# OmerKerner/noLZSS

Measured on AMD Instinct MI355X. Metric: bases/sec factorized (1 GB sigma=4 DNA) + HBM GB/s fraction, higher is better.
Workload: dtype u32; 1 GPU; dna1g: one 2^30-base synthetic DNA sequence per GPU (sigma=4, 40% copied blocks, 1% substitutions), full factorization to (start,length,ref) records in HBM; bases_per_gpu=1073741824, parallelism=1 independent sequence shard(s), all-gather of counts

## Files before the change

nolzss_amd/csrc/lpnf.hip:

```cpp
#include "pipeline.hpp"

#include <cstdlib>
#include "nearest_lds.hpp"
#include "queues.hpp"
#include "text_order.hpp"
#include "scan.hpp"

namespace nolzss {

__global__ void shard_totals_kernel(const uint32_t *const *counts, int nq, uint32_t *totals) {
    const int q = blockIdx.x;
    if (q >= nq) return;
    uint32_t v = threadIdx.x < kQShards ? counts[q][threadIdx.x * kQPad] : 0u;
    v = wave_reduce(v, OpAdd<uint32_t>());
    __shared__ uint32_t s_part[kQShards / 64];
    if (lane_id() == 0) s_part[threadIdx.x >> 6] = v;
    __syncthreads();
    if (threadIdx.x == 0) {
        uint32_t t = 0;
        for (uint32_t k = 0; k < kQShards / 64; ++k) t += s_part[k];
        totals[q] = t;
    }
}

namespace {

constexpr int kThreads = 256;
constexpr uint32_t kFarBothUnknown = 0xfffffffeu;

__device__ __forceinline__ bool lpf_decide(uint32_t i, uint32_t lp, uint32_t jp, uint32_t ls, uint32_t js,
                                           uint32_t *__restrict__ dst) {
    const uint32_t M = lp > ls ? lp : ls;
    if (M == 0) {
        *dst = 0;
        return false;
    }
    const bool ok = (lp == M && i - jp >= M) || (ls == M && i - js >= M);
    if (ok) {
        *dst = M;
        return false;
    }
    uint32_t lo = 0;
    if (lp > 0) { const uint32_t c = lp < i - jp ? lp : i - jp; lo = c > lo ? c : lo; }
    if (ls > 0) { const uint32_t c = ls < i - js ? ls : i - js; lo = c > lo ? c : lo; }
    *dst = lo;
    return true;
}

template <bool kTimed>
__global__ __launch_bounds__(kLdsThreads) void lpf_tile_kernel(const uint32_t *__restrict__ sa,
                                                               const uint32_t *__restrict__ lcp, uint32_t n,
                                                               uint32_t *__restrict__ lstar_by_rank,
                                                               ShardQueue exact_q, uint32_t *__restrict__ far_items,
                                                               uint32_t *__restrict__ far_cnt,
                                                               uint32_t *__restrict__ far_aux,
                                                               unsigned long long *__restrict__ phases,
                                                               uint32_t *__restrict__ psa1, uint32_t *__restrict__ plcp1,
                                                               uint32_t pending_min, uint32_t *__restrict__ pending_flag) {
    constexpr int NS = 2;
    const bool timed = kTimed && phases != nullptr && (blockIdx.x & 15) == 0;
    unsigned long long clk[6] = {0, 0, 0, 0, 0, 0};
    if (timed) clk[0] = __builtin_readcyclecounter();
    __shared__ __align__(16) uint32_t s_sa[kLdsSpan];
    __shared__ __align__(16) uint32_t s_lcp[kLdsSpan + 4];
    __shared__ uint32_t s_len[NS * kLdsTile];
    __shared__ uint16_t s_pos[NS * kLdsTile];
    constexpr int kListCapB = 64;
    __shared__ uint16_t s_list0[kLdsWaves][NS * kLdsPerWave];
    __shared__ uint16_t s_list1[kLdsWaves][NS * kListCapB];
    __shared__ uint32_t s_blk[3 * kBlkTableLen];
    const uint32_t base = blockIdx.x * (uint32_t)kLdsTile;
    const uint32_t shard = blockIdx.x % kQShards;
    stage_tile(sa, lcp, n, base, s_sa, s_lcp, pending_min, pending_flag);
    __syncthreads();
    const BlockTables T = block_tables<false>(s_blk);
    build_block_tables<false>(s_sa, s_lcp, T);
    __syncthreads();
    if (psa1 != nullptr && threadIdx.x < kLdsTile / kBlk) {
        const uint32_t B = (uint32_t)kLdsReach / kBlk + threadIdx.x;
        const uint64_t first = (uint64_t)base + (uint64_t)threadIdx.x * kBlk;
        if (first + kBlk <= (uint64_t)n) {
            psa1[first >> 4] = T.mn[B];
            plcp1[first >> 4] = T.ldn[B];
        }
    }
    if (timed) clk[1] = __builtin_readcyclecounter();
    const int w = threadIdx.x >> 6;
    const uint32_t far_bit = n <= 0x80000000u ? 0x80000000u : 0u;
    lds_search_wave_blocks<NS, NS, false, kLdsPerWave, kListCapB>(s_sa, s_lcp, T, n, base, s_len, s_pos, s_list0[w], s_list1[w],
                                   [](uint32_t) { return true; }, [](uint32_t) { return 0u; }, far_bit,
                                   timed ? clk + 2 : nullptr);
    if (timed) clk[4] = __builtin_readcyclecounter();
    constexpr int kRows = kLdsPerWave / 64;
    bool far[kRows], exact[kRows];
    uint32_t aux[kRows], known[kRows], fslot[kRows], eslot[kRows];
#pragma unroll
    for (int row = 0; row < kRows; ++row) {
        const int t = w * kLdsPerWave + row * 64 + lane_id();
        const uint64_t rr = (uint64_t)base + t;
        const bool in = rr < n;
        uint32_t up = s_len[t], down = s_len[kLdsTile + t];
        const bool fu = far_is(up, far_bit), fd = far_is(down, far_bit);
        far[row] = far_resolve(up, down, far_bit, 0u) && in;
        exact[row] = false;
        aux[row] = kFarBothUnknown;
        known[row] = 0;
        if (far[row]) {
            if (far_bit && fu != fd) {
                known[row] = fu ? down : up;
                const uint32_t p = match_pos(s_sa, fu ? s_pos[kLdsTile + t] : s_pos[t]);
                aux[row] = (known[row] ? (p & 0x7fffffffu) : 0x7fffffffu) | (fu ? 0x80000000u : 0u);
            }
        } else if (in) {
            exact[row] = lpf_decide(s_sa[t + kLdsReach], up, match_pos(s_sa, s_pos[t]), down, match_pos(s_sa, s_pos[kLdsTile + t]),
                                    lstar_by_rank + rr);
        }
    }
    {
        const uint32_t region = (blockIdx.x * (uint32_t)kLdsWaves + (uint32_t)w);
        uint32_t used = 0;
#pragma unroll
        for (int row = 0; row < kRows; ++row) {
            const uint64_t bal = __ballot(far[row]);
            fslot[row] = region * (uint32_t)kLdsPerWave + used + (uint32_t)__popcll(bal & lanemask_lt());
            used += (uint32_t)__popcll(bal);
        }
        if (lane_id() == 0) far_cnt[region] = used;
    }
    shard_slots<kRows>(exact_q, shard, exact, eslot);
#pragma unroll
    for (int row = 0; row < kRows; ++row) {
        const int t = w * kLdsPerWave + row * 64 + lane_id();
        const uint64_t rr = (uint64_t)base + t;
        if (far[row]) {
            far_items[fslot[row]] = (uint32_t)rr;
            lstar_by_rank[rr] = known[row];
            far_aux[rr] = aux[row];
        }
        if (exact[row]) exact_q.items[eslot[row]] = s_sa[t + kLdsReach];
    }
    if (timed) {
        __builtin_amdgcn_s_waitcnt(0);
        clk[5] = __builtin_readcyclecounter();
        if (lane_id() == 0) {
            for (int k = 0; k < 5; ++k) atomicAdd(phases + k, clk[k + 1] - clk[k]);
            atomicAdd(phases + 5, 1ull);
        }
    }
}

__global__ __launch_bounds__(kThreads) void compact_far_kernel(const uint32_t *__restrict__ far_items,
                                                               const uint32_t *__restrict__ far_cnt,
                                                               const uint32_t *__restrict__ far_off, uint32_t regions,
                                                               uint32_t *__restrict__ far_list) {
    const size_t stride = (size_t)gridDim.x * blockDim.x / 4;
    for (size_t r = ((size_t)blockIdx.x * blockDim.x + threadIdx.x) / 4; r < regions; r += stride) {
        const uint32_t c = far_cnt[r], o = far_off[r];
        for (uint32_t k = threadIdx.x & 3u; k < c; k += 4) far_list[o + k] = far_items[r * (size_t)kLdsPerWave + k];
    }
}

__global__ __launch_bounds__(kThreads) void lpf_far_kernel(const uint32_t *__restrict__ far_list, uint32_t far_count,
                                                           const uint32_t *__restrict__ sa,
                                                           const uint32_t *__restrict__ lcp, uint32_t n,
                                                           Pyramid Psa, Pyramid Plcp,
                                                           const uint32_t *__restrict__ by_rank,
                                                           const uint32_t *__restrict__ far_aux, bool bounded,
                                                           uint32_t *__restrict__ lstar, uint32_t *__restrict__ far_exact) {
    const size_t stride = (size_t)gridDim.x * blockDim.x;
    for (size_t k = (size_t)blockIdx.x * blockDim.x + threadIdx.x; k < far_count; k += stride) {
        const uint32_t r = far_list[k];
        const uint32_t i = sa[r];
        const uint32_t aux = far_aux[r];
        uint32_t lp, jp, ls, js;
        if (!bounded) {
            nearest_up<false>(sa, lcp, Psa, Plcp, r, i, 0u, lp, jp);
            nearest_down<false>(sa, lcp, n, Psa, Plcp, r, i, lp, ls, js);
        } else if (aux == kFarBothUnknown) {
            far_up<false>(sa, Psa, Plcp, r, i, 0u, lp, jp);
            far_down<false>(sa, n, Psa, Plcp, r, i, lp, ls, js);
        } else if (aux >> 31) {
            ls = by_rank[r];
            js = (aux & 0x7fffffffu) == 0x7fffffffu ? kNoPos : (aux & 0x7fffffffu);
            far_up<false>(sa, Psa, Plcp, r, i, ls, lp, jp);
        } else {
            lp = by_rank[r];
            jp = (aux & 0x7fffffffu) == 0x7fffffffu ? kNoPos : (aux & 0x7fffffffu);
            far_down<false>(sa, n, Psa, Plcp, r, i, lp, ls, js);
        }
        far_exact[k] = lpf_decide(i, lp, jp, ls, js, lstar + i) ? i : kNoPos;
    }
}

__global__ __launch_bounds__(kThreads) void lpnf_fallback_list_kernel(const uint32_t *__restrict__ far_exact,
                                                                      uint32_t far_count, uint32_t n,
                                                                      const uint32_t *__restrict__ isa, Pyramid Psa,
                                                                      Pyramid Plcp, uint32_t *__restrict__ lstar) {
    const size_t stride = (size_t)gridDim.x * blockDim.x;
    for (size_t k = (size_t)blockIdx.x * blockDim.x + threadIdx.x; k < far_count; k += stride) {
        const uint32_t i = far_exact[k];
        if (i == kNoPos) continue;
        const uint32_t cap = (n - i) < i ? (n - i) : i;
        lstar[i] = lpnf_search(Psa, Plcp, isa[i] - 1u, i, lstar[i], cap);
    }
}

__global__ __launch_bounds__(kThreads) void lpnf_fallback_kernel(ShardQueue exact_q, uint32_t n,
                                                                 const uint32_t *__restrict__ isa,
                                                                 Pyramid Psa, Pyramid Plcp,
                                                                 uint32_t *__restrict__ lstar) {
    const uint32_t shard = blockIdx.x;
    const uint32_t count = exact_q.counts[shard * kQPad];
    const uint32_t *items = exact_q.items + (size_t)shard * exact_q.cap;
    for (uint32_t k = blockIdx.y * blockDim.x + threadIdx.x; k < count; k += gridDim.y * blockDim.x) {
        const uint32_t i = items[k];
        const uint32_t cap = (n - i) < i ? (n - i) : i;
        lstar[i] = lpnf_search(Psa, Plcp, isa[i] - 1u, i, lstar[i], cap);
    }
}

}

uint32_t build_lstar(Context &ctx, uint32_t n, const uint32_t *sa, const uint32_t *isa, const uint32_t *lcp,
                     const Pyramid &Psa, const Pyramid &Plcp, uint32_t *lstar, uint32_t *isa_fill,
                     const PackedText *fill_pyramids) {
    hipStream_t s = ctx.stream;
    const size_t mark = ctx.arena.mark();
    uint32_t *pending_flag = nullptr;
    if (fill_pyramids) {
        pending_flag = ctx.arena.alloc<uint32_t>(1);
        HIP_CHECK(hipMemsetAsync(pending_flag, 0, sizeof(uint32_t), s));
        inject_pending_for_test(ctx, const_cast<uint32_t *>(lcp), n);
    }
    uint32_t *psa1 = fill_pyramids && Psa.nlev > 1 ? const_cast<uint32_t *>(Psa.lvl[1]) : nullptr;
    uint32_t *plcp1 = fill_pyramids && Plcp.nlev > 1 ? const_cast<uint32_t *>(Plcp.lvl[1]) : nullptr;
    if (!psa1 || !plcp1) psa1 = plcp1 = nullptr;
    const unsigned tiles = (unsigned)div_up(n, kLdsTile);
    ShardQueue exact_q;
    exact_q.cap = (uint32_t)shard_queue_cap(tiles, kLdsTile);
    exact_q.items = ctx.arena.alloc<uint32_t>((size_t)kQShards * exact_q.cap);
    const uint32_t far_regions = tiles * (uint32_t)kLdsWaves;
    uint32_t *far_items = ctx.arena.alloc<uint32_t>((size_t)far_regions * kLdsPerWave);
    uint32_t *far_cnt = ctx.arena.alloc<uint32_t>(far_regions);
    uint32_t *far_off = ctx.arena.alloc<uint32_t>(far_regions);
    uint32_t *qcounts = ctx.arena.alloc<uint32_t>(kQShards * kQPad);
    exact_q.counts = qcounts;
    const uint32_t **count_ptrs = ctx.arena.alloc<const uint32_t *>(1);
    uint32_t *totals = ctx.arena.alloc<uint32_t>(2);
    uint32_t *by_rank = ctx.arena.alloc<uint32_t>(n);
    uint32_t *far_aux = ctx.arena.alloc<uint32_t>(n);
    uint32_t *scratch_idx = ctx.arena.alloc<uint32_t>(n);
    uint32_t *scratch_val = ctx.arena.alloc<uint32_t>(isa_fill ? 2 * (size_t)n : (size_t)n);
    HIP_CHECK(hipMemsetAsync(qcounts, 0, kQShards * kQPad * sizeof(uint32_t), s));
    const uint32_t *h_ptrs[1] = {exact_q.counts};
    HIP_CHECK(hipMemcpyAsync(count_ptrs, h_ptrs, sizeof h_ptrs, hipMemcpyHostToDevice, s));
    HIP_CHECK(hipStreamSynchronize(s));
    auto read_totals = [&](uint32_t h[2]) {
        shard_totals_kernel<<<1, kQShards, 0, s>>>(count_ptrs, 1, totals);
        KERNEL_CHECK();
        ctx.read_back(totals, h, 2);
    };
    {
        ProfScope ps(ctx.profiler(), "lpf", s, 12.0 * (double)n);
        static const bool want_phases = getenv("NOLZSS_LPF_PHASES") != nullptr;
        unsigned long long *phases = nullptr;
        if (want_phases) {
            phases = ctx.arena.alloc<unsigned long long>(8);
            HIP_CHECK(hipMemsetAsync(phases, 0, 64, s));
        }
        if (phases)
            lpf_tile_kernel<true><<<tiles, kLdsThreads, 0, s>>>(sa, lcp, n, by_rank, exact_q, far_items, far_cnt, far_aux, phases, psa1, plcp1,
                                                                pending_threshold(), pending_flag);
        else
            lpf_tile_kernel<false><<<tiles, kLdsThreads, 0, s>>>(sa, lcp, n, by_rank, exact_q, far_items, far_cnt, far_aux, nullptr, psa1,
                                                                 plcp1, pending_threshold(), pending_flag);
        KERNEL_CHECK();
        if (phases) {
            unsigned long long h[8];
            HIP_CHECK(hipMemcpyAsync(h, phases, 64, hipMemcpyDeviceToHost, s));
            HIP_CHECK(hipStreamSynchronize(s));
            const double w = h[5] ? (double)h[5] : 1.0;
            fprintf(stderr, "[nolzss] lpf_tile phases (cycles per wavefront, %llu sampled): stage %.0f  round0 %.0f  %s %.0f  %s %.0f  epilogue %.0f\n",
                    h[5], h[0] / w, h[1] / w, "roundA", h[2] / w, "roundsBC", h[3] / w, h[4] / w);
        }
    }
    scan_exclusive_add_u32(far_cnt, far_off, far_regions, totals + 1, ctx.arena, s);
    if (fill_pyramids) {
        ProfScope ps(ctx.profiler(), "pyramids", s);
        if (psa1) {
            fill_pyramid_tail(Psa, n >> kPyrShift, false, s);
            fill_pyramid_tail(Plcp, n >> kPyrShift, false, s);
            fill_pyramid(Psa, 2, false, s);
            fill_pyramid(Plcp, 2, false, s);
        } else {
            fill_pyramid(Psa, 1, false, s);
            fill_pyramid(Plcp, 1, false, s);
        }
        uint32_t pending = 0;
        ctx.read_back(pending_flag, &pending, 1);
        if (pending) {
            ctx.arena.rewind(mark);
            finish_pending_lcp(ctx, *fill_pyramids, sa, const_cast<uint32_t *>(lcp));
            fill_pyramid(Psa, 1, false, s);
            fill_pyramid(Plcp, 1, false, s);
            return build_lstar(ctx, n, sa, isa, lcp, Psa, Plcp, lstar, isa_fill, nullptr);
        }
    }
    {
        ProfScope ps(ctx.profiler(), "lpf_to_text_order", s);
        uint32_t *idx[2] = {const_cast<uint32_t *>(sa), scratch_idx};
        uint32_t *val[2] = {by_rank, scratch_val};
        bucketed_scatter(idx, val, n, lstar, n, ctx.arena, s, ctx.profiler(), true, true, ctx.rec_plan, isa_fill);
    }
    uint32_t h[2] = {0, 0};
    read_totals(h);
    static const bool trace = getenv("NOLZSS_TRACE") != nullptr;
    if (trace) fprintf(stderr, "[nolzss] lpf: %u ranks to the far queue, %u positions to the exact search so far\n", h[1], h[0]);
    if (h[1] > 0) {
        ProfScope ps(ctx.profiler(), "lpf_far", s);
        uint32_t *far_list = ctx.arena.alloc<uint32_t>(h[1]);
        compact_far_kernel<<<(unsigned)std::min<size_t>(div_up((size_t)far_regions * 4, kThreads), 256u * 16u), kThreads, 0, s>>>(
            far_items, far_cnt, far_off, far_regions, far_list);
        KERNEL_CHECK();
        uint32_t *far_exact = ctx.arena.alloc<uint32_t>(h[1]);
        const unsigned g = (unsigned)std::min<size_t>(256u * 64u, std::max<size_t>(1, div_up(h[1], kThreads)));
        lpf_far_kernel<<<g, kThreads, 0, s>>>(far_list, h[1], sa, lcp, n, Psa, Plcp, by_rank, far_aux, n <= 0x80000000u,
                                              lstar, far_exact);
        KERNEL_CHECK();
        lpnf_fallback_list_kernel<<<g, kThreads, 0, s>>>(far_exact, h[1], n, isa, Psa, Plcp, lstar);
        KERNEL_CHECK();
    }
    if (h[0] > 0) {
        ProfScope ps(ctx.profiler(), "lpnf_fallback", s);
        const unsigned gy = (unsigned)std::min<size_t>(64, std::max<size_t>(1, div_up(h[0], (size_t)kQShards * kThreads)));
        lpnf_fallback_kernel<<<dim3(kQShards, gy), kThreads, 0, s>>>(exact_q, n, isa, Psa, Plcp, lstar);
        KERNEL_CHECK();
    }
    ctx.arena.rewind(mark);
    return h[0];
}

}
```

nolzss_amd/csrc/nearest_lds.hpp:

```cpp
#pragma once
#include "nearest.hpp"

#include <type_traits>

namespace nolzss {

constexpr int kLdsThreads = 256;
constexpr int kLdsWaves = kLdsThreads / 64;
constexpr int kLdsTile = 1024;
constexpr int kLdsPerWave = kLdsTile / kLdsWaves;
constexpr int kLdsReach = 256;
constexpr int kLdsSpan = kLdsTile + 2 * kLdsReach;
constexpr int kLdsStep0 = 4;
constexpr uint32_t kFarLen = 0xffffffffu;
__device__ __forceinline__ uint32_t far_mark(uint32_t m, uint32_t far_bit) {
    return far_bit ? (far_bit | (m & ~far_bit)) : kFarLen;
}
__device__ __forceinline__ bool far_is(uint32_t v, uint32_t far_bit) {
    return far_bit ? (v & far_bit) != 0 : v == kFarLen;
}
__device__ __forceinline__ uint32_t far_bound(uint32_t v, uint32_t far_bit) {
    return far_bit ? (v & ~far_bit) : 0xffffffffu;
}
__device__ __forceinline__ bool far_resolve(uint32_t &up, uint32_t &down, uint32_t far_bit, uint32_t floor_len) {
// ... 38 lines not shown
    }
    if (pending) atomicOr(flag, 1u);
}

constexpr uint16_t kNoMatch = 0xffffu;
__device__ __forceinline__ uint32_t match_pos(const uint32_t *s_sa, uint16_t at) { return at == kNoMatch ? kNoPos : s_sa[at]; }
template <int kSteps, bool kGreater, bool kUp>
__device__ __forceinline__ int lds_scan_round(const uint32_t *s_sa, const uint32_t *s_lcp, int li, int s0, uint32_t x,
                                              uint32_t &m, uint32_t &at) {
    uint32_t c[kSteps], v[kSteps];
#pragma unroll
    for (int k = 0; k < kSteps; ++k) {
        const int q = kUp ? li - (s0 + k + 1) : li + (s0 + k + 1);
        c[k] = s_lcp[q + (kUp ? 1 : 0)];
        v[k] = s_sa[q];
    }
    bool alive = true;
    uint32_t kk = 0;
#pragma unroll
    for (int k = 0; k < kSteps; ++k) {
        const uint32_t mk = c[k] < m ? c[k] : m;
        const bool qual = kGreater ? v[k] > x : v[k] < x;
        const bool stop = alive && qual;
        m = alive ? mk : m;
        kk = stop ? (uint32_t)k : kk;
        alive = alive != stop;
    }
    at = (uint32_t)(kUp ? li - (s0 + (int)kk + 1) : li + (s0 + (int)kk + 1));
    return m == 0 ? 0 : (alive ? 2 : 1);
}

constexpr int kBlk = 16;
constexpr int kNumBlk = kLdsSpan / kBlk;
static_assert(kLdsSpan % kBlk == 0 && kLdsReach % kBlk == 0 && kLdsTile % kBlk == 0, "aligned blocks");
constexpr int kStepA = 12;
static_assert(kLdsStep0 + kStepA + 1 >= kBlk, "round B would look at the rank itself and at ranks on its other side");

constexpr int kBlkTableLen = kNumBlk + 2;
struct BlockTables {
    uint32_t *mn, *mx;
    uint32_t *lup, *ldn;
};
template <bool kMax> __device__ __forceinline__ BlockTables block_tables(uint32_t *mem) {
    if (kMax) return BlockTables{mem + 1, mem + kBlkTableLen + 1, mem + 2 * kBlkTableLen + 1, mem + 3 * kBlkTableLen + 1};
    return BlockTables{mem + 1, nullptr, mem + kBlkTableLen + 1, mem + 2 * kBlkTableLen + 1};
}

template <bool kMax>
__device__ __forceinline__ void build_block_tables(const uint32_t *s_sa, const uint32_t *s_lcp, const BlockTables &T) {
    const int B = (int)threadIdx.x;
    if (B < kNumBlk) {
        const uint4 *p = reinterpret_cast<const uint4 *>(s_sa + kBlk * B);
        const uint4 *c = reinterpret_cast<const uint4 *>(s_lcp + kBlk * B);
        uint32_t mn = 0xffffffffu, mx = 0u, lo = 0xffffffffu;
        uint32_t first = 0;
#pragma unroll
        for (int q = 0; q < 4; ++q) {
            const uint4 a = p[q], l = c[q];
            const uint32_t av[4] = {a.x, a.y, a.z, a.w}, lv[4] = {l.x, l.y, l.z, l.w};
#pragma unroll
            for (int e = 0; e < 4; ++e) {
                mn = av[e] < mn ? av[e] : mn;
                mx = av[e] > mx ? av[e] : mx;
                if (q == 0 && e == 0)
                    first = lv[e];
                else
                    lo = lv[e] < lo ? lv[e] : lo;
            }
        }
        const uint32_t last = s_lcp[kBlk * B + kBlk];
        T.mn[B] = mn;
        if (kMax) T.mx[B] = mx;
        T.ldn[B] = lo < first ? lo : first;
        T.lup[B] = lo < last ? lo : last;
    } else if (B < kNumBlk + 2) {
        const int o = B == kNumBlk ? -1 : kNumBlk;
        T.mn[o] = 0xffffffffu;
        if (kMax) T.mx[o] = 0u;
        T.ldn[o] = 0xffffffffu;
        T.lup[o] = 0xffffffffu;
    }
}

constexpr uint32_t kListOverflow = 0xffffffffu;
template <bool kGreater, bool kUp, bool kHasPos, int kListCapB, typename ThrGt>
__device__ __forceinline__ void lds_search_tail(const uint32_t *s_sa, const uint32_t *s_lcp, const BlockTables &T, int w,
                                                uint32_t *res_len, uint16_t *res_pos, const uint16_t *list, uint32_t cnt,
                                                uint16_t *list_b, ThrGt thr_gt, uint32_t far_bit) {
    static_assert(kListCapB >= 64, "a step of round A appends up to 64 searches");
    const int lane = lane_id();
    const uint64_t lt = lanemask_lt();
    const uint32_t *tv = kGreater ? T.mx : T.mn;
    const uint32_t *tc = kUp ? T.lup : T.ldn;
    auto rounds_bc = [&](uint32_t cnt_b) {
        __builtin_amdgcn_fence(__ATOMIC_RELEASE, "wavefront");
        __builtin_amdgcn_wave_barrier();
        for (uint32_t c0 = 0; c0 < cnt_b; c0 += 64) {
            const bool have = c0 + lane < cnt_b;
            const int tl = have ? (int)list_b[c0 + lane] : 0;
            const int t = w * kLdsPerWave + tl;
            const int li = t + kLdsReach;
            const uint32_t i = s_sa[li];
            const uint32_t x = kGreater ? thr_gt(i) : i;
            const int b0 = kUp ? (li - (kLdsStep0 + kStepA + 1)) >> 4 : (li + (kLdsStep0 + kStepA + 1)) >> 4;
            uint32_t c[kBlk], v[kBlk];
#pragma unroll
            for (int j = 0; j < kBlk; ++j) {
                const int B = kUp ? b0 - j : b0 + j;
                c[j] = tc[B];
                v[j] = tv[B];
            }
            uint32_t run = have ? res_len[t] : 0xffffffffu;
            int jstar = -1;
            bool alive = true;
#pragma unroll
            for (int j = 0; j < kBlk; ++j) {
                const uint32_t rk = c[j] < run ? c[j] : run;
                const bool qual = kGreater ? v[j] > x : v[j] < x;
                const bool stop = alive && qual;
                jstar = stop ? j : jstar;
                alive = alive != stop;
                run = alive ? rk : run;
            }
            const bool inside = have && jstar >= 0;
            const int Bs = kUp ? b0 - jstar : b0 + jstar;
            const int anchor = inside ? (kUp ? kBlk * Bs + kBlk : kBlk * Bs - 1) : li;
            uint32_t m = run, at = 0;
            const int st = lds_scan_round<kBlk, kGreater, kUp>(s_sa, s_lcp, anchor, 0, x, m, at);
            if (have) {
                res_len[t] = inside ? m : far_mark(run, far_bit);
                if (kHasPos) res_pos[t] = (inside && st == 1) ? (uint16_t)at : kNoMatch;
            }
        }
        __builtin_amdgcn_fence(__ATOMIC_RELEASE, "wavefront");
        __builtin_amdgcn_wave_barrier();
    };
    uint32_t cnt_b = 0;
    for (uint32_t c0 = 0; c0 < cnt; c0 += 64) {
        if (kListCapB < kLdsPerWave && cnt_b + 64 > (uint32_t)kListCapB) {
            rounds_bc(cnt_b);
            cnt_b = 0;
        }
        const bool have = c0 + lane < cnt;
        const int tl = have ? (int)list[c0 + lane] : 0;
        const int t = w * kLdsPerWave + tl;
        const int li = t + kLdsReach;
        bool pending = false;
        if (have) {
            const uint32_t i = s_sa[li];
            uint32_t m = res_len[t], at = 0;
            const int st = lds_scan_round<kStepA, kGreater, kUp>(s_sa, s_lcp, li, kLdsStep0, kGreater ? thr_gt(i) : i, m, at);
            pending = st == 2;
            res_len[t] = m;
            if (kHasPos) res_pos[t] = (st == 1) ? (uint16_t)at : kNoMatch;
        }
        const uint64_t bal = __ballot(pending);
        if (pending) list_b[cnt_b + (uint32_t)__popcll(bal & lt)] = (uint16_t)tl;
        cnt_b += (uint32_t)__popcll(bal);
    }
    rounds_bc(cnt_b);
}

template <int NS, int NP, bool kCompact = false, int kListCap = kLdsPerWave, int kListCapB = kListCap, typename Active, typename ThrGt>
__device__ __forceinline__ void lds_search_wave_blocks(const uint32_t *s_sa, const uint32_t *s_lcp,
                                                       const BlockTables &T, uint32_t n, uint32_t base,
                                                       uint32_t *res_len, uint16_t *res_pos, uint16_t *list0,
                                                       uint16_t *list1, Active active, ThrGt thr_gt,
                                                       uint32_t far_bit, unsigned long long *phase_clock = nullptr) {
    static_assert(NS == 2 || NS == 4, "searches: smaller up / down, then greater up / down");
    const int lane = lane_id();
    const int w = threadIdx.x >> 6;
    const uint64_t lt = lanemask_lt();
    uint32_t cnt[NS];
#pragma unroll
    for (int k = 0; k < NS; ++k) cnt[k] = 0;

    uint32_t rows = kLdsPerWave / 64, n_act = kLdsPerWave;
    if (kCompact) {
        n_act = 0;
#pragma unroll
        for (int row = 0; row < kLdsPerWave / 64; ++row) {
            const int tl = row * 64 + lane;
            const int t = w * kLdsPerWave + tl;
            const bool valid = (uint64_t)base + t < n && active(s_sa[t + kLdsReach]);
            const uint64_t bal = __ballot(valid);
            if (valid) list1[n_act + (uint32_t)__popcll(bal & lt)] = (uint16_t)tl;
            n_act += (uint32_t)__popcll(bal);
        }
        __builtin_amdgcn_fence(__ATOMIC_RELEASE, "wavefront");
        __builtin_amdgcn_wave_barrier();
        rows = (n_act + 63) / 64;
    }
#pragma unroll 1
    for (uint32_t row = 0; row < rows; ++row) {
        const bool have = !kCompact || row * 64 + lane < n_act;
        const int tl = kCompact ? (have ? (int)list1[row * 64 + lane] : 0) : (int)(row * 64 + lane);
        const int t = w * kLdsPerWave + tl;
        const uint64_t rr = (uint64_t)base + t;
        const int li = t + kLdsReach;
        const uint32_t i = s_sa[li];
        const bool valid = kCompact ? have : (rr < n && active(i));
        auto search = [&](auto kk) {
            constexpr int k = decltype(kk)::value;
            constexpr bool greater = k >= 2, up = (k & 1) == 0;
            uint32_t m = 0xffffffffu, at = 0;
            int st = 0;
            if (valid) st = lds_scan_round<kLdsStep0, greater, up>(s_sa, s_lcp, li, 0, greater ? thr_gt(i) : i, m, at);
            if (have) {
                res_len[k * kLdsTile + t] = (st == 0) ? 0u : m;
                if (k < NP) res_pos[k * kLdsTile + t] = (st == 1) ? (uint16_t)at : kNoMatch;
            }
            const bool pending = st == 2;
            const uint64_t bal = __ballot(pending);
            const uint32_t slot = cnt[k] + (uint32_t)__popcll(bal & lt);
            if (pending) {
                if (kListCap >= kLdsPerWave || slot < (uint32_t)kListCap)
                    list0[k * kListCap + slot] = (uint16_t)tl;
                else
                    res_len[k * kLdsTile + t] = kListOverflow;
            }
            cnt[k] += (uint32_t)__popcll(bal);
            if (kListCap < kLdsPerWave && cnt[k] > (uint32_t)kListCap) cnt[k] = (uint32_t)kListCap;
        };
        search(std::integral_constant<int, 0>());
        search(std::integral_constant<int, 1>());
        if constexpr (NS > 2) {
            search(std::integral_constant<int, 2>());
            search(std::integral_constant<int, 3>());
        }
    }
    if (phase_clock) phase_clock[0] = __builtin_readcyclecounter();
    __builtin_amdgcn_fence(__ATOMIC_RELEASE, "wavefront");
    __builtin_amdgcn_wave_barrier();

    static_assert(!kCompact || NS * kListCapB >= kLdsPerWave, "list1 first holds the gathered ranks");
    lds_search_tail<false, true, (0 < NP), kListCapB>(s_sa, s_lcp, T, w, res_len, res_pos, list0, cnt[0], list1, thr_gt, far_bit);
    lds_search_tail<false, false, (1 < NP), kListCapB>(s_sa, s_lcp, T, w, res_len + kLdsTile, res_pos + kLdsTile, list0 + kListCap,
                                                       cnt[1], list1 + kListCapB, thr_gt, far_bit);
    if constexpr (NS > 2) {
        lds_search_tail<true, true, (2 < NP), kListCapB>(s_sa, s_lcp, T, w, res_len + 2 * kLdsTile, res_pos + (2 < NP ? 2 : 0) * kLdsTile,
                                                         list0 + 2 * kListCap, cnt[2], list1 + 2 * kListCapB, thr_gt, far_bit);
        lds_search_tail<true, false, (3 < NP), kListCapB>(s_sa, s_lcp, T, w, res_len + 3 * kLdsTile, res_pos + (3 < NP ? 3 : 0) * kLdsTile,
                                                          list0 + 3 * kListCap, cnt[3], list1 + 3 * kListCapB, thr_gt, far_bit);
    }
    if (phase_clock) phase_clock[1] = phase_clock[2] = __builtin_readcyclecounter();
    __builtin_amdgcn_fence(__ATOMIC_RELEASE, "wavefront");
    __builtin_amdgcn_wave_barrier();
}

}
```

nolzss_amd/csrc/rc.hip:

```cpp
#include <algorithm>

#include "nearest_lds.hpp"
#include "pipeline.hpp"
#include "queues.hpp"
#include "text_order.hpp"
#include "scan.hpp"

namespace nolzss {
namespace {

constexpr int kThreads = 256;
constexpr uint32_t kRcFlag = 0x80000000u;

__device__ __forceinline__ uint32_t rc_select(uint32_t fwd, uint32_t rc) {
    if (fwd >= 1) return (rc > fwd) ? (rc | kRcFlag) : fwd;
    return (rc > 1) ? (rc | kRcFlag) : 0u;
}

template <bool kPlain>
__device__ __forceinline__ bool rc_decide(uint32_t i, uint32_t lp, uint32_t jp, uint32_t ls, uint32_t js,
                                          uint32_t rc, uint32_t *__restrict__ dst, uint32_t *__restrict__ plain) {
    const uint32_t M = lp > ls ? lp : ls;
    const bool fwd_final = (M == 0) || (lp == M && i - jp >= M) || (ls == M && i - js >= M);
    if (fwd_final) {
        *dst = rc_select(M, rc);
        if (kPlain) *plain = M;
        return false;
    }
    uint32_t lo = 0;
    if (lp > 0) { const uint32_t c = lp < i - jp ? lp : i - jp; lo = c > lo ? c : lo; }
    if (ls > 0) { const uint32_t c = ls < i - js ? ls : i - js; lo = c > lo ? c : lo; }
    *dst = lo;
    if (kPlain) *plain = lo;
    return true;
}

template <bool kPlain>
__global__ __launch_bounds__(kLdsThreads) void rc_tile_kernel(const uint32_t *__restrict__ sa,
                                                              const uint32_t *__restrict__ lcp, uint32_t m,
                                                              uint32_t N, uint32_t *__restrict__ code_by_rank,
                                                              ShardQueue exact_q, ShardQueue far_q,
                                                              uint32_t *__restrict__ pmin1, uint32_t *__restrict__ pmax1,
                                                              uint32_t *__restrict__ plcp1, uint32_t pending_min,
                                                              uint32_t *__restrict__ pending_flag,
                                                              const uint32_t *__restrict__ tile_off,
                                                              uint32_t *__restrict__ cidx, uint64_t *__restrict__ cpacked,
                                                              uint32_t *__restrict__ plain_by_rank) {
    constexpr int NS = 4, NP = 2;
    __shared__ __align__(16) uint32_t s_sa[kLdsSpan];
    __shared__ __align__(16) uint32_t s_lcp[kLdsSpan + 4];
    __shared__ uint32_t s_len[NS * kLdsTile];
    __shared__ uint16_t s_pos[NP * kLdsTile];
    constexpr int kListCap = 128;
    constexpr int kListCapB = 64;
    __shared__ uint16_t s_list0[kLdsWaves][NS * kListCap];
    __shared__ uint16_t s_list1[kLdsWaves][NS * kListCapB];
    __shared__ uint32_t s_blk[4 * kBlkTableLen];
    const uint32_t base = blockIdx.x * (uint32_t)kLdsTile;
    const uint32_t shard = blockIdx.x % kQShards;
    stage_tile(sa, lcp, m, base, s_sa, s_lcp, pending_min, pending_flag);
    __syncthreads();
    const BlockTables T = block_tables<true>(s_blk);
    build_block_tables<true>(s_sa, s_lcp, T);
    __syncthreads();
    if (pmin1 != nullptr && threadIdx.x < kLdsTile / kBlk) {
        const uint32_t B = (uint32_t)kLdsReach / kBlk + threadIdx.x;
        const uint64_t first = (uint64_t)base + (uint64_t)threadIdx.x * kBlk;
        if (first + kBlk <= (uint64_t)m) {
            pmin1[first >> 4] = T.mn[B];
            pmax1[first >> 4] = T.mx[B];
            plcp1[first >> 4] = T.ldn[B];
        }
    }
    const int w = threadIdx.x >> 6;
    const uint32_t far_bit = m <= 0x80000000u ? 0x80000000u : 0u;
    lds_search_wave_blocks<NS, NP, true, kListCap, kListCapB>(s_sa, s_lcp, T, m, base, s_len, s_pos, s_list0[w], s_list1[w],
                                   [N](uint32_t i) { return i < N; }, [N](uint32_t i) { return 2u * N - i; }, far_bit);
    constexpr int kRows = kLdsPerWave / 64;
    bool far[kRows], exact[kRows];
    uint32_t mask[kRows], rcl[kRows], fslot[kRows], eslot[kRows];
    const bool compact_out = cidx != nullptr;
    uint32_t cbase = 0;
    if (compact_out) {
        uint32_t before = 0;
        for (int t2 = lane_id(); t2 < w * kLdsPerWave; t2 += 64)
            before += ((uint64_t)base + t2 < m && s_sa[t2 + kLdsReach] < N) ? 1u : 0u;
        cbase = tile_off[blockIdx.x] + wave_reduce(before, OpAdd<uint32_t>());
    }
    uint32_t cv[kRows], cat[kRows];
#pragma unroll
    for (int row = 0; row < kRows; ++row) {
        const int t = w * kLdsPerWave + row * 64 + lane_id();
        const uint64_t rr = (uint64_t)base + t;
        const uint32_t i = s_sa[t + kLdsReach];
        far[row] = exact[row] = false;
        mask[row] = rcl[row] = 0;
        cv[row] = 0;
        const bool orig = rr < m && i < N;
        {
            const uint64_t ob = __ballot(orig);
            cat[row] = orig ? cbase + (uint32_t)__popcll(ob & lanemask_lt()) : 0xffffffffu;
            cbase += (uint32_t)__popcll(ob);
        }
        if (rr >= m) continue;
        if (i >= N) {
            if (!compact_out) code_by_rank[rr] = 0;
            continue;
        }
        uint32_t lp = s_len[t], ls = s_len[kLdsTile + t];
        uint32_t ru = s_len[2 * kLdsTile + t], rd = s_len[3 * kLdsTile + t];
        if (far_bit)
            mask[row] = ((far_is(lp, far_bit) && lp != kListOverflow) ? 1u : 0u) | ((far_is(ls, far_bit) && ls != kListOverflow) ? 2u : 0u) |
                        ((far_is(ru, far_bit) && ru != kListOverflow) ? 4u : 0u) | ((far_is(rd, far_bit) && rd != kListOverflow) ? 8u : 0u);
        const bool far_f = far_resolve(lp, ls, far_bit, 0u);
        const bool far_r = far_resolve(ru, rd, far_bit, 1u);
        far[row] = far_f || far_r;
        if (!far[row]) {
            rcl[row] = ru > rd ? ru : rd;
            uint32_t pv = 0;
            exact[row] = rc_decide<kPlain>(i, lp, match_pos(s_sa, s_pos[t]), ls, match_pos(s_sa, s_pos[kLdsTile + t]), rcl[row],
                                           &cv[row], &pv);
            if (!compact_out) code_by_rank[rr] = cv[row];
            if (kPlain) plain_by_rank[rr] = pv;
        }
    }
    shard_slots<kRows>(far_q, shard, far, fslot);
    shard_slots<kRows>(exact_q, shard, exact, eslot);
#pragma unroll
    for (int row = 0; row < kRows; ++row) {
        const int t = w * kLdsPerWave + row * 64 + lane_id();
        const uint64_t rr = (uint64_t)base + t;
        if (far[row]) {
            far_q.items[fslot[row]] = (uint32_t)rr;
            code_by_rank[rr] = mask[row];
        }
        if (exact[row]) {
            exact_q.items[eslot[row]] = s_sa[t + kLdsReach];
            exact_q.items2[eslot[row]] = rcl[row];
        }
        if (compact_out && cat[row] != 0xffffffffu) {
            cidx[cat[row]] = s_sa[t + kLdsReach];
            cpacked[cat[row]] = (uint64_t)cv[row] | ((uint64_t)((uint32_t)rr + 1u) << 32);
        }
    }
}

__global__ __launch_bounds__(kLdsThreads) void rc_count_original_kernel(const uint32_t *__restrict__ sa, uint32_t m, uint32_t N,
                                                                        uint32_t *__restrict__ counts) {
    const size_t base = (size_t)blockIdx.x * kLdsTile;
    uint32_t c = 0;
#pragma unroll
    for (int k = 0; k < kLdsTile / kLdsThreads; ++k) {
        const size_t r = base + (size_t)k * kLdsThreads + threadIdx.x;
        c += (r < m && sa[r < m ? r : m - 1] < N) ? 1u : 0u;
    }
    c = wave_reduce(c, OpAdd<uint32_t>());
    __shared__ uint32_t s_part[kLdsWaves];
    if (lane_id() == 0) s_part[threadIdx.x >> 6] = c;
    __syncthreads();
// ... 351 lines not shown
```

Measured before the change: 13.17 billion bases/s.

## Pool rounds B/C search lists across all waves of a tile

Instead of each wavefront finishing its own leftover B/C searches, per-wave leftover counts are published to LDS and after a block barrier all four waves process the concatenated lists of the tile round-robin. This balances uneven per-wave work and improves lane utilisation for sparse lists, at the cost of two extra __syncthreads per tile and cross-wave indexing. A per-wave fallback kernel selectable by environment variable and extended phase/occupancy instrumentation are also added, and the timed sampling rate is reduced.

New measurement: 13.27 billion bases/s, median of 6. About the same (+0.8%).

```diff
diff --git a/nolzss_amd/csrc/lpnf.hip b/nolzss_amd/csrc/lpnf.hip
--- a/nolzss_amd/csrc/lpnf.hip
+++ b/nolzss_amd/csrc/lpnf.hip
@@ -47,19 +47,18 @@
     return true;
 }
 
-template <bool kTimed>
-__global__ __launch_bounds__(kLdsThreads) void lpf_tile_kernel(const uint32_t *__restrict__ sa,
-                                                               const uint32_t *__restrict__ lcp, uint32_t n,
-                                                               uint32_t *__restrict__ lstar_by_rank,
-                                                               ShardQueue exact_q, uint32_t *__restrict__ far_items,
-                                                               uint32_t *__restrict__ far_cnt,
-                                                               uint32_t *__restrict__ far_aux,
-                                                               unsigned long long *__restrict__ phases,
-                                                               uint32_t *__restrict__ psa1, uint32_t *__restrict__ plcp1,
-                                                               uint32_t pending_min, uint32_t *__restrict__ pending_flag) {
+constexpr int kLpfPhaseWords = 16;
+template <bool kTimed, bool kPool>
+__device__ __forceinline__ void lpf_tile_body(const uint32_t *__restrict__ sa, const uint32_t *__restrict__ lcp, uint32_t n,
+                                              uint32_t *__restrict__ lstar_by_rank, ShardQueue exact_q,
+                                              uint32_t *__restrict__ far_items, uint32_t *__restrict__ far_cnt,
+                                              uint32_t *__restrict__ far_aux, unsigned long long *__restrict__ phases,
+                                              uint32_t *__restrict__ psa1, uint32_t *__restrict__ plcp1, uint32_t pending_min,
+                                              uint32_t *__restrict__ pending_flag) {
     constexpr int NS = 2;
-    const bool timed = kTimed && phases != nullptr && (blockIdx.x & 15) == 0;
-    unsigned long long clk[6] = {0, 0, 0, 0, 0, 0};
+    const bool timed = kTimed && phases != nullptr && (blockIdx.x & 1023) == 0;
+    unsigned long long clk[4] = {0, 0, 0, 0};
+    SearchClocks ck;
     if (timed) clk[0] = __builtin_readcyclecounter();
     __shared__ __align__(16) uint32_t s_sa[kLdsSpan];
     __shared__ __align__(16) uint32_t s_lcp[kLdsSpan + 4];
@@ -68,6 +67,7 @@
     constexpr int kListCapB = 64;
     __shared__ uint16_t s_list0[kLdsWaves][NS * kLdsPerWave];
     __shared__ uint16_t s_list1[kLdsWaves][NS * kListCapB];
+    __shared__ uint32_t s_pool[NS * kLdsWaves];
     __shared__ uint32_t s_blk[3 * kBlkTableLen];
     const uint32_t base = blockIdx.x * (uint32_t)kLdsTile;
     const uint32_t shard = blockIdx.x % kQShards;
@@ -87,10 +87,10 @@
     if (timed) clk[1] = __builtin_readcyclecounter();
     const int w = threadIdx.x >> 6;
     const uint32_t far_bit = n <= 0x80000000u ? 0x80000000u : 0u;
-    lds_search_wave_blocks<NS, NS, false, kLdsPerWave, kListCapB>(s_sa, s_lcp, T, n, base, s_len, s_pos, s_list0[w], s_list1[w],
-                                   [](uint32_t) { return true; }, [](uint32_t) { return 0u; }, far_bit,
-                                   timed ? clk + 2 : nullptr);
-    if (timed) clk[4] = __builtin_readcyclecounter();
+    lds_search_wave_blocks<NS, NS, false, kLdsPerWave, kListCapB, kPool>(s_sa, s_lcp, T, n, base, s_len, s_pos, s_list0[w], s_list1[0],
+                                   s_pool, [](uint32_t) { return true; }, [](uint32_t) { return 0u; }, far_bit,
+                                   kTimed ? &ck : nullptr);
+    if (timed) clk[2] = __builtin_readcyclecounter();
     constexpr int kRows = kLdsPerWave / 64;
     bool far[kRows], exact[kRows];
     uint32_t aux[kRows], known[kRows], fslot[kRows], eslot[kRows];
@@ -141,13 +141,30 @@
     }
     if (timed) {
         __builtin_amdgcn_s_waitcnt(0);
-        clk[5] = __builtin_readcyclecounter();
+        clk[3] = __builtin_readcyclecounter();
         if (lane_id() == 0) {
-            for (int k = 0; k < 5; ++k) atomicAdd(phases + k, clk[k + 1] - clk[k]);
-            atomicAdd(phases + 5, 1ull);
-        }
-    }
-}
+            const unsigned long long v[14] = {clk[1] - clk[0], ck.round0_end - clk[1], ck.round_a, ck.bc_wave, ck.wait, ck.bc_pool,
+                                              clk[3] - clk[2], 1ull, ck.n_list0, ck.n_bc_wave, ck.it_bc_wave, ck.n_left, ck.n_pool,
+                                              ck.it_pool};
+            for (int k = 0; k < 14; ++k) atomicAdd(phases + k, v[k]);
+        }
+    }
+}
+
+#define NOLZSS_LPF_TILE_PARAMS                                                                                               \
+    const uint32_t *__restrict__ sa, const uint32_t *__restrict__ lcp, uint32_t n, uint32_t *__restrict__ lstar_by_rank,       \
+        ShardQueue exact_q, uint32_t *__restrict__ far_items, uint32_t *__restrict__ far_cnt, uint32_t *__restrict__ far_aux, \
+        unsigned long long *__restrict__ phases, uint32_t *__restrict__ psa1, uint32_t *__restrict__ plcp1,                   \
+        uint32_t pending_min, uint32_t *__restrict__ pending_flag
+#define NOLZSS_LPF_TILE_ARGS sa, lcp, n, lstar_by_rank, exact_q, far_items, far_cnt, far_aux, phases, psa1, plcp1, pending_min, pending_flag
+template <bool kTimed> __global__ __launch_bounds__(kLdsThreads) void lpf_tile_kernel(NOLZSS_LPF_TILE_PARAMS) {
+    lpf_tile_body<kTimed, true>(NOLZSS_LPF_TILE_ARGS);
+}
+template <bool kTimed> __global__ __launch_bounds__(kLdsThreads) void lpf_tile_perwave_kernel(NOLZSS_LPF_TILE_PARAMS) {
+    lpf_tile_body<kTimed, false>(NOLZSS_LPF_TILE_ARGS);
+}
+#undef NOLZSS_LPF_TILE_PARAMS
+#undef NOLZSS_LPF_TILE_ARGS
 
 __global__ __launch_bounds__(kThreads) void compact_far_kernel(const uint32_t *__restrict__ far_items,
                                                                const uint32_t *__restrict__ far_cnt,
@@ -263,25 +280,30 @@
     {
         ProfScope ps(ctx.profiler(), "lpf", s, 12.0 * (double)n);
         static const bool want_phases = getenv("NOLZSS_LPF_PHASES") != nullptr;
+        static const bool per_wave = getenv("NOLZSS_LPF_PER_WAVE") != nullptr;
         unsigned long long *phases = nullptr;
         if (want_phases) {
-            phases = ctx.arena.alloc<unsigned long long>(8);
-            HIP_CHECK(hipMemsetAsync(phases, 0, 64, s));
-        }
-        if (phases)
-            lpf_tile_kernel<true><<<tiles, kLdsThreads, 0, s>>>(sa, lcp, n, by_rank, exact_q, far_items, far_cnt, far_aux, phases, psa1, plcp1,
-                                                                pending_threshold(), pending_flag);
-        else
-            lpf_tile_kernel<false><<<tiles, kLdsThreads, 0, s>>>(sa, lcp, n, by_rank, exact_q, far_items, far_cnt, far_aux, nullptr, psa1,
-                                                                 plcp1, pending_threshold(), pending_flag);
+            phases = ctx.arena.alloc<unsigned long long>(kLpfPhaseWords);
+            HIP_CHECK(hipMemsetAsync(phases, 0, kLpfPhaseWords * sizeof(unsigned long long), s));
+        }
+        auto *kernel = phases ? (per_wave ? lpf_tile_perwave_kernel<true> : lpf_tile_kernel<true>)
+                              : (per_wave ? lpf_tile_perwave_kernel<false> : lpf_tile_kernel<false>);
+        kernel<<<tiles, kLdsThreads, 0, s>>>(sa, lcp, n, by_rank, exact_q, far_items, far_cnt, far_aux, phases, psa1, plcp1,
+                                             pending_threshold(), pending_flag);
         KERNEL_CHECK();
         if (phases) {
-            unsigned long long h[8];
-            HIP_CHECK(hipMemcpyAsync(h, phases, 64, hipMemcpyDeviceToHost, s));
+            unsigned long long h[kLpfPhaseWords];
+            HIP_CHECK(hipMemcpyAsync(h, phases, sizeof h, hipMemcpyDeviceToHost, s));
             HIP_CHECK(hipStreamSynchronize(s));
-            const double w = h[5] ? (double)h[5] : 1.0;
-            fprintf(stderr, "[nolzss] lpf_tile phases (cycles per wavefront, %llu sampled): stage %.0f  round0 %.0f  %s %.0f  %s %.0f  epilogue %.0f\n",
-                    h[5], h[0] / w, h[1] / w, "roundA", h[2] / w, "roundsBC", h[3] / w, h[4] / w);
+            const double w = h[7] ? (double)h[7] : 1.0;
+            auto fill = [](unsigned long long entries, unsigned long long iters) { return iters ? (double)entries / (64.0 * (double)iters) : 0.0; };
+            fprintf(stderr, "[nolzss] lpf_tile phases (%s finish; cycles per wavefront, %llu sampled): stage %.0f  round0 %.0f  roundA %.0f  "
+                            "roundsBC_wave %.0f  barriers %.0f  roundsBC_pool %.0f  epilogue %.0f\n",
+                    per_wave ? "per-wave" : "pooled", h[7], h[0] / w, h[1] / w, h[2] / w, h[3] / w, h[4] / w, h[5] / w, h[6] / w);
+            fprintf(stderr, "[nolzss] lpf_tile lists (per wavefront): round-A lists %.1f entries  per-wave B+C %.1f entries in %.2f iterations "
+                            "(lane use %.2f)  left for the pool %.1f  pooled lists of the tile %.1f entries, %.2f iterations per wavefront "
+                            "(lane use %.2f)\n",
+                    h[8] / w, h[9] / w, h[10] / w, fill(h[9], h[10]), h[11] / w, h[12] / w, h[13] / w, fill(h[11], h[13]));
         }
     }
     scan_exclusive_add_u32(far_cnt, far_off, far_regions, totals + 1, ctx.arena, s);
diff --git a/nolzss_amd/csrc/nearest_lds.hpp b/nolzss_amd/csrc/nearest_lds.hpp
--- a/nolzss_amd/csrc/nearest_lds.hpp
+++ b/nolzss_amd/csrc/nearest_lds.hpp
@@ -144,58 +144,88 @@
     }
 }
 
+struct SearchClocks {
+    unsigned long long round0_end = 0;
+    unsigned long long round_a = 0;
+    unsigned long long bc_wave = 0;
+    unsigned long long wait = 0;
+    unsigned long long bc_pool = 0;
+    uint32_t n_list0 = 0;
+    uint32_t n_bc_wave = 0, it_bc_wave = 0;
+    uint32_t n_left = 0;
+    uint32_t n_pool = 0, it_pool = 0;
+};
+
+template <bool kGreater, bool kUp, bool kHasPos, typename ThrGt>
+__device__ __forceinline__ void lds_rounds_bc(const uint32_t *s_sa, const uint32_t *s_lcp, const BlockTables &T, bool have, int t,
+                                              uint32_t *res_len, uint16_t *res_pos, ThrGt thr_gt, uint32_t far_bit) {
+    const uint32_t *tv = kGreater ? T.mx : T.mn;
+    const uint32_t *tc = kUp ? T.lup : T.ldn;
+    const int li = t + kLdsReach;
+    const uint32_t i = s_sa[li];
+    const uint32_t x = kGreater ? thr_gt(i) : i;
+    const int b0 = kUp ? (li - (kLdsStep0 + kStepA + 1)) >> 4 : (li + (kLdsStep0 + kStepA + 1)) >> 4;
+    uint32_t c[kBlk], v[kBlk];
+#pragma unroll
+    for (int j = 0; j < kBlk; ++j) {
+        const int B = kUp ? b0 - j : b0 + j;
+        c[j] = tc[B];
+        v[j] = tv[B];
+    }
+    uint32_t run = have ? res_len[t] : 0xffffffffu;
+    int jstar = -1;
+    bool alive = true;
+#pragma unroll
+    for (int j = 0; j < kBlk; ++j) {
+        const uint32_t rk = c[j] < run ? c[j] : run;
+        const bool qual = kGreater ? v[j] > x : v[j] < x;
+        const bool stop = alive && qual;
+        jstar = stop ? j : jstar;
+        alive = alive != stop;
+        run = alive ? rk : run;
+    }
+    const bool inside = have && jstar >= 0;
+    const int Bs = kUp ? b0 - jstar : b0 + jstar;
+    const int anchor = inside ? (kUp ? kBlk * Bs + kBlk : kBlk * Bs - 1) : li;
+    uint32_t m = run, at = 0;
+    const int st = lds_scan_round<kBlk, kGreater, kUp>(s_sa, s_lcp, anchor, 0, x, m, at);
+    if (have) {
+        res_len[t] = inside ? m : far_mark(run, far_bit);
+        if (kHasPos) res_pos[t] = (inside && st == 1) ? (uint16_t)at : kNoMatch;
+    }
+}
+
 constexpr uint32_t kListOverflow = 0xffffffffu;
-template <bool kGreater, bool kUp, bool kHasPos, int kListCapB, typename ThrGt>
-__device__ __forceinline__ void lds_search_tail(const uint32_t *s_sa, const uint32_t *s_lcp, const BlockTables &T, int w,
-                                                uint32_t *res_len, uint16_t *res_pos, const uint16_t *list, uint32_t cnt,
-                                                uint16_t *list_b, ThrGt thr_gt, uint32_t far_bit) {
+template <bool kGreater, bool kUp, bool kHasPos, int kListCapB, bool kPool, typename ThrGt>
+__device__ __forceinline__ uint32_t lds_search_tail(const uint32_t *s_sa, const uint32_t *s_lcp, const BlockTables &T, int w,
+                                                    uint32_t *res_len, uint16_t *res_pos, const uint16_t *list, uint32_t cnt,
+                                                    uint16_t *list_b, ThrGt thr_gt, uint32_t far_bit, SearchClocks *ck) {
     static_assert(kListCapB >= 64, "a step of round A appends up to 64 searches");
     const int lane = lane_id();
     const uint64_t lt = lanemask_lt();
-    const uint32_t *tv = kGreater ? T.mx : T.mn;
-    const uint32_t *tc = kUp ? T.lup : T.ldn;
+    unsigned long long t0 = ck ? __builtin_readcyclecounter() : 0ull;
     auto rounds_bc = [&](uint32_t cnt_b) {
+        if (ck) {
+            const unsigned long long t1 = __builtin_readcyclecounter();
+            ck->round_a += t1 - t0;
+            t0 = t1;
+            ck->n_bc_wave += cnt_b;
+            ck->it_bc_wave += (cnt_b + 63) / 64;
+        }
         __builtin_amdgcn_fence(__ATOMIC_RELEASE, "wavefront");
         __builtin_amdgcn_wave_barrier();
         for (uint32_t c0 = 0; c0 < cnt_b; c0 += 64) {
             const bool have = c0 + lane < cnt_b;
             const int tl = have ? (int)list_b[c0 + lane] : 0;
-            const int t = w * kLdsPerWave + tl;
-            const int li = t + kLdsReach;
-            const uint32_t i = s_sa[li];
-            const uint32_t x = kGreater ? thr_gt(i) : i;
-            const int b0 = kUp ? (li - (kLdsStep0 + kStepA + 1)) >> 4 : (li + (kLdsStep0 + kStepA + 1)) >> 4;
-            uint32_t c[kBlk], v[kBlk];
-#pragma unroll
-            for (int j = 0; j < kBlk; ++j) {
-                const int B = kUp ? b0 - j : b0 + j;
-                c[j] = tc[B];
-                v[j] = tv[B];
-            }
-            uint32_t run = have ? res_len[t] : 0xffffffffu;
-            int jstar = -1;
-            bool alive = true;
-#pragma unroll
-            for (int j = 0; j < kBlk; ++j) {
-                const uint32_t rk = c[j] < run ? c[j] : run;
-                const bool qual = kGreater ? v[j] > x : v[j] < x;
-                const bool stop = alive && qual;
-                jstar = stop ? j : jstar;
-                alive = alive != stop;
-                run = alive ? rk : run;
-            }
-            const bool inside = have && jstar >= 0;
-            const int Bs = kUp ? b0 - jstar : b0 + jstar;
-            const int anchor = inside ? (kUp ? kBlk * Bs + kBlk : kBlk * Bs - 1) : li;
-            uint32_t m = run, at = 0;
-            const int st = lds_scan_round<kBlk, kGreater, kUp>(s_sa, s_lcp, anchor, 0, x, m, at);
-            if (have) {
-                res_len[t] = inside ? m : far_mark(run, far_bit);
-                if (kHasPos) res_pos[t] = (inside && st == 1) ? (uint16_t)at : kNoMatch;
-            }
+            lds_rounds_bc<kGreater, kUp, kHasPos>(s_sa, s_lcp, T, have, w * kLdsPerWave + tl, res_len, res_pos, thr_gt, far_bit);
         }
         __builtin_amdgcn_fence(__ATOMIC_RELEASE, "wavefront");
         __builtin_amdgcn_wave_barrier();
+        if (ck) {
+            const unsigned long long t1 = __builtin_readcyclecounter();
+            ck->bc_wave += t1 - t0;
+            t0 = t1;
+        }
     };
     uint32_t cnt_b = 0;
     for (uint32_t c0 = 0; c0 < cnt; c0 += 64) {
@@ -220,19 +250,53 @@
         if (pending) list_b[cnt_b + (uint32_t)__popcll(bal & lt)] = (uint16_t)tl;
         cnt_b += (uint32_t)__popcll(bal);
     }
-    rounds_bc(cnt_b);
-}
-
-template <int NS, int NP, bool kCompact = false, int kListCap = kLdsPerWave, int kListCapB = kListCap, typename Active, typename ThrGt>
+    if (!kPool) {
+        rounds_bc(cnt_b);
+        cnt_b = 0;
+    } else if (ck) {
+        ck->round_a += __builtin_readcyclecounter() - t0;
+    }
+    return cnt_b;
+}
+
+template <int k, int NS, int NP, int kListCapB, typename ThrGt>
+__device__ __forceinline__ void lds_pool_finish(const uint32_t *s_sa, const uint32_t *s_lcp, const BlockTables &T, int w,
+                                                uint32_t *res_len, uint16_t *res_pos, const uint16_t *list1_tile,
+                                                const uint32_t *pool_cnt, ThrGt thr_gt, uint32_t far_bit, SearchClocks *ck) {
+    static_assert(kLdsWaves == 4, "three prefix sums");
+    constexpr bool greater = k >= 2, up = (k & 1) == 0;
+    const int lane = lane_id();
+    const uint32_t p1 = (uint32_t)__builtin_amdgcn_readfirstlane((int)pool_cnt[k * kLdsWaves]);
+    const uint32_t p2 = p1 + (uint32_t)__builtin_amdgcn_readfirstlane((int)pool_cnt[k * kLdsWaves + 1]);
+    const uint32_t p3 = p2 + (uint32_t)__builtin_amdgcn_readfirstlane((int)pool_cnt[k * kLdsWaves + 2]);
+    const uint32_t total = p3 + (uint32_t)__builtin_amdgcn_readfirstlane((int)pool_cnt[k * kLdsWaves + 3]);
+    if (ck) ck->n_pool += total;
+    const int ws = __builtin_amdgcn_readfirstlane(w);
+    for (uint32_t c0 = 64u * (uint32_t)((ws - k * (kLdsWaves / NS)) & (kLdsWaves - 1)); c0 < total; c0 += 64u * kLdsWaves) {
+        const uint32_t idx = c0 + (uint32_t)lane;
+        const bool have = idx < total;
+        const uint32_t v = have ? (idx >= p1 ? 1u : 0u) + (idx >= p2 ? 1u : 0u) + (idx >= p3 ? 1u : 0u) : 0u;
+        const uint32_t pre = v == 0 ? 0u : (v == 1 ? p1 : (v == 2 ? p2 : p3));
+        const uint32_t e = have ? idx - pre : 0u;
+        const int tl = (int)list1_tile[v * (uint32_t)(NS * kListCapB) + (uint32_t)(k * kListCapB) + e];
+        lds_rounds_bc<greater, up, (k < NP)>(s_sa, s_lcp, T, have, have ? (int)v * kLdsPerWave + tl : 0, res_len + k * kLdsTile,
+                                             res_pos + (k < NP ? k : 0) * kLdsTile, thr_gt, far_bit);
+        if (ck) ck->it_pool += 1;
+    }
+}
+
+template <int NS, int NP, bool kCompact = false, int kListCap = kLdsPerWave, int kListCapB = kListCap, bool kPool = false,
+          typename Active, typename ThrGt>
 __device__ __forceinline__ void lds_search_wave_blocks(const uint32_t *s_sa, const uint32_t *s_lcp,
                                                        const BlockTables &T, uint32_t n, uint32_t base,
                                                        uint32_t *res_len, uint16_t *res_pos, uint16_t *list0,
-                                                       uint16_t *list1, Active active, ThrGt thr_gt,
-                                                       uint32_t far_bit, unsigned long long *phase_clock = nullptr) {
+                                                       uint16_t *list1_tile, uint32_t *pool_cnt, Active active, ThrGt thr_gt,
+                                                       uint32_t far_bit, SearchClocks *ck = nullptr) {
     static_assert(NS == 2 || NS == 4, "searches: smaller up / down, then greater up / down");
     const int lane = lane_id();
     const int w = threadIdx.x >> 6;
     const uint64_t lt = lanemask_lt();
+    uint16_t *list1 = list1_tile + w * (NS * kListCapB);
     uint32_t cnt[NS];
 #pragma unroll
     for (int k = 0; k < NS; ++k) cnt[k] = 0;
@@ -291,23 +355,62 @@
             search(std::integral_constant<int, 3>());
         }
     }
-    if (phase_clock) phase_clock[0] = __builtin_readcyclecounter();
+    if (ck) {
+        ck->round0_end = __builtin_readcyclecounter();
+#pragma unroll
+        for (int k = 0; k < NS; ++k) ck->n_list0 += cnt[k];
+    }
     __builtin_amdgcn_fence(__ATOMIC_RELEASE, "wavefront");
     __builtin_amdgcn_wave_barrier();
 
     static_assert(!kCompact || NS * kListCapB >= kLdsPerWave, "list1 first holds the gathered ranks");
-    lds_search_tail<false, true, (0 < NP), kListCapB>(s_sa, s_lcp, T, w, res_len, res_pos, list0, cnt[0], list1, thr_gt, far_bit);
-    lds_search_tail<false, false, (1 < NP), kListCapB>(s_sa, s_lcp, T, w, res_len + kLdsTile, res_pos + kLdsTile, list0 + kListCap,
-                                                       cnt[1], list1 + kListCapB, thr_gt, far_bit);
+    uint32_t left[NS];
+    left[0] = lds_search_tail<false, true, (0 < NP), kListCapB, kPool>(s_sa, s_lcp, T, w, res_len, res_pos, list0, cnt[0], list1, thr_gt,
+                                                                       far_bit, ck);
+    left[1] = lds_search_tail<false, false, (1 < NP), kListCapB, kPool>(s_sa, s_lcp, T, w, res_len + kLdsTile, res_pos + kLdsTile,
+                                                                        list0 + kListCap, cnt[1], list1 + kListCapB, thr_gt, far_bit, ck);
     if constexpr (NS > 2) {
-        lds_search_tail<true, true, (2 < NP), kListCapB>(s_sa, s_lcp, T, w, res_len + 2 * kLdsTile, res_pos + (2 < NP ? 2 : 0) * kLdsTile,
-                                                         list0 + 2 * kListCap, cnt[2], list1 + 2 * kListCapB, thr_gt, far_bit);
-        lds_search_tail<true, false, (3 < NP), kListCapB>(s_sa, s_lcp, T, w, res_len + 3 * kLdsTile, res_pos + (3 < NP ? 3 : 0) * kLdsTile,
-                                                          list0 + 3 * kListCap, cnt[3], list1 + 3 * kListCapB, thr_gt, far_bit);
-    }
-    if (phase_clock) phase_clock[1] = phase_clock[2] = __builtin_readcyclecounter();
-    __builtin_amdgcn_fence(__ATOMIC_RELEASE, "wavefront");
-    __builtin_amdgcn_wave_barrier();
-}
-
-}
+        left[2] = lds_search_tail<true, true, (2 < NP), kListCapB, kPool>(s_sa, s_lcp, T, w, res_len + 2 * kLdsTile,
+                                                                          res_pos + (2 < NP ? 2 : 0) * kLdsTile, list0 + 2 * kListCap, cnt[2],
+                                                                          list1 + 2 * kListCapB, thr_gt, far_bit, ck);
+        left[3] = lds_search_tail<true, false, (3 < NP), kListCapB, kPool>(s_sa, s_lcp, T, w, res_len + 3 * kLdsTile,
+                                                                           res_pos + (3 < NP ? 3 : 0) * kLdsTile, list0 + 3 * kListCap, cnt[3],
+                                                                           list1 + 3 * kListCapB, thr_gt, far_bit, ck);
+    }
+    if constexpr (!kPool) {
+        __builtin_amdgcn_fence(__ATOMIC_RELEASE, "wavefront");
+        __builtin_amdgcn_wave_barrier();
+    } else {
+        if (lane == 0) {
+#pragma unroll
+            for (int k = 0; k < NS; ++k) pool_cnt[k * kLdsWaves + w] = left[k];
+        }
+        unsigned long long t0 = 0;
+        if (ck) {
+            t0 = __builtin_readcyclecounter();
+#pragma unroll
+            for (int k = 0; k < NS; ++k) ck->n_left += left[k];
+        }
+        __syncthreads();
+        if (ck) {
+            const unsigned long long t1 = __builtin_readcyclecounter();
+            ck->wait += t1 - t0;
+            t0 = t1;
+        }
+        lds_pool_finish<0, NS, NP, kListCapB>(s_sa, s_lcp, T, w, res_len, res_pos, list1_tile, pool_cnt, thr_gt, far_bit, ck);
+        lds_pool_finish<1, NS, NP, kListCapB>(s_sa, s_lcp, T, w, res_len, res_pos, list1_tile, pool_cnt, thr_gt, far_bit, ck);
+        if constexpr (NS > 2) {
+            lds_pool_finish<2, NS, NP, kListCapB>(s_sa, s_lcp, T, w, res_len, res_pos, list1_tile, pool_cnt, thr_gt, far_bit, ck);
+            lds_pool_finish<3, NS, NP, kListCapB>(s_sa, s_lcp, T, w, res_len, res_pos, list1_tile, pool_cnt, thr_gt, far_bit, ck);
+        }
+        if (ck) {
+            const unsigned long long t1 = __builtin_readcyclecounter();
+            ck->bc_pool += t1 - t0;
+            t0 = t1;
+        }
+        __syncthreads();
+        if (ck) ck->wait += __builtin_readcyclecounter() - t0;
+    }
+}
+
+}
diff --git a/nolzss_amd/csrc/rc.hip b/nolzss_amd/csrc/rc.hip
--- a/nolzss_amd/csrc/rc.hip
+++ b/nolzss_amd/csrc/rc.hip
@@ -55,6 +55,7 @@
     constexpr int kListCapB = 64;
     __shared__ uint16_t s_list0[kLdsWaves][NS * kListCap];
     __shared__ uint16_t s_list1[kLdsWaves][NS * kListCapB];
+    __shared__ uint32_t s_pool[NS * kLdsWaves];
     __shared__ uint32_t s_blk[4 * kBlkTableLen];
     const uint32_t base = blockIdx.x * (uint32_t)kLdsTile;
     const uint32_t shard = blockIdx.x % kQShards;
@@ -74,7 +75,7 @@
     }
     const int w = threadIdx.x >> 6;
     const uint32_t far_bit = m <= 0x80000000u ? 0x80000000u : 0u;
-    lds_search_wave_blocks<NS, NP, true, kListCap, kListCapB>(s_sa, s_lcp, T, m, base, s_len, s_pos, s_list0[w], s_list1[w],
+    lds_search_wave_blocks<NS, NP, true, kListCap, kListCapB, true>(s_sa, s_lcp, T, m, base, s_len, s_pos, s_list0[w], s_list1[0], s_pool,
                                    [N](uint32_t i) { return i < N; }, [N](uint32_t i) { return 2u * N - i; }, far_bit);
     constexpr int kRows = kLdsPerWave / 64;
     bool far[kRows], exact[kRows];
```
